# imisumi/software-path-tracer

Hardware: AMD Instinct MI355X
Metric: Msamples/sec (whole node), 1920x1080 x 8-bounce Cornell box (higher is better)
Workload: dtype f32

## Files before the change

include/spt.h:

```cpp
#ifndef SPT_H
#define SPT_H

#include <stddef.h>
#include <stdint.h>

#ifdef __cplusplus
extern "C" {
#endif

#define SPT_ABI_VERSION 3

typedef enum spt_status {
    SPT_OK = 0,
    SPT_ERR_INVALID = -1,
    SPT_ERR_HIP = -2,
    SPT_ERR_NO_DEVICE = -3,
    SPT_ERR_NO_SCENE = -4,
    SPT_ERR_NOT_CONFIGURED = -5,
    SPT_ERR_CAPACITY = -6
} spt_status;


typedef enum spt_prim_type {
    SPT_PRIM_SPHERE = 0,
// ... 40 lines not shown

typedef struct spt_config {
    uint32_t width;
    uint32_t height;
    uint32_t max_bounces;
    uint32_t rr_depth;
    uint32_t flags;
    uint32_t shard_rank;
    uint32_t shard_count;
    uint32_t frames_in_flight;
} spt_config;

#define SPT_MAX_BOUNCES 32
typedef struct spt_stats {
    uint64_t frames;
    uint64_t paths;
    uint64_t segments[SPT_MAX_BOUNCES];
    uint64_t segments_total;
    uint64_t passes;
    uint64_t extend_launches;
    double extend_ms;
    uint64_t extend_segments;
    uint64_t shade_launches;
    double shade_ms;
    double other_ms;
    double extend_ms_bounce[SPT_MAX_BOUNCES];
    double shade_ms_bounce[SPT_MAX_BOUNCES];
    uint64_t bvh_nodes;
    uint64_t scene_bytes;
    uint64_t radiance_updates[SPT_MAX_BOUNCES];
    double tail_ms;
    uint64_t tail_launches;
    uint64_t tail_bounce;
    uint64_t fused;
    double persistent_ms;
    uint64_t persistent_launches;
    uint64_t schedule;
    uint64_t lane_slots;
    uint64_t lane_busy;
    uint64_t bvh_node_visits;
    uint64_t prim_tests;
    uint64_t flat_fast_path;
    uint64_t specialized;
    uint64_t shadow_rays;
    uint64_t emitters;
    uint64_t stack_bytes;
    uint64_t stack_need;
    uint64_t stalled_waves;
    uint64_t view_cached;
    uint64_t view_live_pixels;
    uint64_t flat_pairs;
    uint64_t flat_pair_second_passes;
    uint64_t view_split;
} spt_stats;

typedef struct spt_ctx spt_ctx;

int spt_abi_version(void);
int spt_device_count(int* count);

int spt_create(spt_ctx** out, int device_id);
void spt_destroy(spt_ctx* ctx);
const char* spt_last_error(const spt_ctx* ctx);
int spt_set_stream(spt_ctx* ctx, void* hip_stream);

int spt_set_scene(spt_ctx* ctx, const spt_prim* prims, uint32_t n_prims,
                  const spt_material* mats, uint32_t n_mats, const spt_env* env);

int spt_update_prims(spt_ctx* ctx, const uint32_t* indices, const spt_prim* prims, uint32_t n);

int spt_configure(spt_ctx* ctx, const spt_config* cfg);
int spt_reset(spt_ctx* ctx);
int spt_get_frame_count(const spt_ctx* ctx, uint32_t* frame_count);

int spt_render(spt_ctx* ctx, uint32_t first_frame, uint32_t n_frames);
int spt_synchronize(spt_ctx* ctx);

int spt_shard_pixels(const spt_ctx* ctx, uint64_t* n_pixels);
int spt_read_accum(spt_ctx* ctx, float* host_rgba);
int spt_accum_device_ptr(spt_ctx* ctx, void** dptr, size_t* bytes);
int spt_copy_accum_device(spt_ctx* ctx, void* dst);
int spt_resolve_rgba8(spt_ctx* ctx, uint32_t frame_count, uint32_t* host_out);
int spt_resolve_rgba8_exposure(spt_ctx* ctx, uint32_t frame_count, float exposure, uint32_t* host_out);
int spt_register_host_output(spt_ctx* ctx, void* host_out, size_t bytes);
int spt_render_resolve_rgba8(spt_ctx* ctx, uint32_t first_frame, uint32_t n_frames, uint32_t frame_count,
                             float exposure, uint32_t* host_out);
int spt_assemble_rows(spt_ctx* ctx, const void* gathered, void* out);

#define SPT_CAMERA_JITTER 1u
typedef struct spt_camera {
    float origin[3], u[3], v[3], w[3];
    uint32_t flags;
    uint32_t reserved[3];
} spt_camera;
int spt_set_camera(spt_ctx* ctx, const spt_camera* camera);
int spt_camera_look_at(const float eye[3], const float target[3], const float up[3], float vfov_degrees,
                       spt_camera* out);
int spt_camera_ray(const spt_camera* camera, uint32_t width, uint32_t height, uint32_t x, uint32_t y,
                   float jx, float jy, float o[3], float d[3]);

typedef struct spt_lens {
    float radius;
    float focus_distance;
    uint32_t reserved[2];
} spt_lens;
int spt_set_camera_lens(spt_ctx* ctx, const spt_lens* lens);
// ... 91 lines not shown
```

software-path-tracer_amd/__init__.py:

```python
from __future__ import annotations

import ctypes
import enum
import os
from typing import Optional, Sequence, Tuple

import numpy as np

_HERE = os.path.dirname(os.path.abspath(__file__))
LIB_PATH = os.environ.get("SPT_LIB_PATH") or os.path.join(_HERE, "libspt_hip.so")
RENDER_LIB_PATH = os.path.join(_HERE, "libspt_render.so")

SPT_OK = 0
SPT_ERR = {
    -1: "SPT_ERR_INVALID",
    -2: "SPT_ERR_HIP",
    -3: "SPT_ERR_NO_DEVICE",
    -4: "SPT_ERR_NO_SCENE",
    -5: "SPT_ERR_NOT_CONFIGURED",
    -6: "SPT_ERR_CAPACITY",
}

PRIM_SPHERE, PRIM_QUAD, PRIM_TRIANGLE = 0, 1, 2
FLAG_ABS_FLOAT = 1
# ... 61 lines not shown
class SptLens(ctypes.Structure):
    _fields_ = [
        ("radius", ctypes.c_float),
        ("focus_distance", ctypes.c_float),
        ("reserved", ctypes.c_uint32 * 2),
    ]


CAMERA_JITTER = 1
SPT_MAX_BOUNCES = 32


class SptStats(ctypes.Structure):
    _fields_ = [
        ("frames", ctypes.c_uint64),
        ("paths", ctypes.c_uint64),
        ("segments", ctypes.c_uint64 * SPT_MAX_BOUNCES),
        ("segments_total", ctypes.c_uint64),
        ("passes", ctypes.c_uint64),
        ("extend_launches", ctypes.c_uint64),
        ("extend_ms", ctypes.c_double),
        ("extend_segments", ctypes.c_uint64),
        ("shade_launches", ctypes.c_uint64),
        ("shade_ms", ctypes.c_double),
        ("other_ms", ctypes.c_double),
        ("extend_ms_bounce", ctypes.c_double * SPT_MAX_BOUNCES),
        ("shade_ms_bounce", ctypes.c_double * SPT_MAX_BOUNCES),
        ("bvh_nodes", ctypes.c_uint64),
        ("scene_bytes", ctypes.c_uint64),
        ("radiance_updates", ctypes.c_uint64 * SPT_MAX_BOUNCES),
        ("tail_ms", ctypes.c_double),
        ("tail_launches", ctypes.c_uint64),
        ("tail_bounce", ctypes.c_uint64),
        ("fused", ctypes.c_uint64),
        ("persistent_ms", ctypes.c_double),
        ("persistent_launches", ctypes.c_uint64),
        ("schedule", ctypes.c_uint64),
        ("lane_slots", ctypes.c_uint64),
        ("lane_busy", ctypes.c_uint64),
        ("bvh_node_visits", ctypes.c_uint64),
        ("prim_tests", ctypes.c_uint64),
        ("flat_fast_path", ctypes.c_uint64),
        ("specialized", ctypes.c_uint64),
        ("shadow_rays", ctypes.c_uint64),
        ("emitters", ctypes.c_uint64),
        ("stack_bytes", ctypes.c_uint64),
        ("stack_need", ctypes.c_uint64),
        ("stalled_waves", ctypes.c_uint64),
        ("view_cached", ctypes.c_uint64),
        ("view_live_pixels", ctypes.c_uint64),
        ("flat_pairs", ctypes.c_uint64),
        ("flat_pair_second_passes", ctypes.c_uint64),
        ("view_split", ctypes.c_uint64),
    ]

    def as_dict(self) -> dict:
        d = {}
        for k, _ in self._fields_:
            v = getattr(self, k)
            d[k] = list(v) if isinstance(v, ctypes.Array) else v
        return d


EXPORTED_SYMBOLS = (
    "spt_abi_version", "spt_device_count", "spt_create", "spt_destroy", "spt_last_error", "spt_set_stream",
    "spt_set_scene", "spt_configure", "spt_reset", "spt_get_frame_count", "spt_render", "spt_synchronize",
    "spt_shard_pixels", "spt_read_accum", "spt_accum_device_ptr", "spt_copy_accum_device", "spt_resolve_rgba8",
    "spt_resolve_rgba8_exposure", "spt_register_host_output", "spt_render_resolve_rgba8", "spt_assemble_rows",
    "spt_set_profiling", "spt_get_stats", "spt_stats_clear", "spt_build_scene",
    "spt_set_env_map", "spt_env_octa_from_equirect",
    "spt_comm_available", "spt_comm_unique_id", "spt_comm_init", "spt_gather_image", "spt_gather_image_overlapped", "spt_gather_wait",
    "spt_comm_destroy", "spt_set_tuning",
    "spt_specialize_scene", "spt_compile_flat_kernels", "spt_update_prims",
    "spt_set_camera", "spt_camera_look_at", "spt_camera_ray",
    "spt_set_camera_lens", "spt_camera_lens_ray", "spt_camera_focus_at_hit",
    "spt_set_material_models", "spt_bsdf_sample",
    "spt_render_features", "spt_read_features", "spt_features_device_ptr",
    "spt_denoise_params_default", "spt_denoise", "spt_set_denoise_form", "spt_read_denoised", "spt_denoised_device_ptr",
    "spt_resolve_denoised_rgba8", "spt_atrous_host",
)
COMM_ID_BYTES = 128


class SptTuning(ctypes.Structure):
    _fields_ = [
        ("fused", ctypes.c_int32),
        ("tail_bounce", ctypes.c_uint32),
        ("persistent", ctypes.c_int32),
        ("frame_kernel", ctypes.c_int32),
        ("chunks_per_wave", ctypes.c_uint32),
        ("px_shift", ctypes.c_uint32),
        ("subqueues", ctypes.c_uint32),
        ("bvh_max_leaf", ctypes.c_uint32),
        ("bvh_bins", ctypes.c_uint32),
        ("specialize", ctypes.c_int32),
        ("view_cache", ctypes.c_int32),
        ("split_streams", ctypes.c_int32),
    ]

    def __init__(self, **kw):
        super().__init__(fused=-1, persistent=-1, frame_kernel=-1)
        for k, v in kw.items():
            if k not in dict(self._fields_):
                raise TypeError(f"unknown spt_tuning field {k}")
            setattr(self, k, v)

# ... 793 lines not shown
```

software-path-tracer_amd/csrc/spt_capi.hip:

```cpp
#include <dlfcn.h>
#include <hip/hip_runtime.h>
#include <rccl/rccl.h>

#include <algorithm>
#include <cmath>
#include <cstdio>
#include <cstdlib>
#include <cstring>
#include <string>
#include <vector>

#include "scene.h"
#include "spt.h"
#include "spt_denoise.h"
#include "spt_device.h"
#include "spt_jit.h"
#include "spt_kernels.h"
#include "spt_launch_plan.h"

using namespace spt;

static_assert(kBvhStackMax == kBvhStackEntries, "scene.h and spt_kernels.h stack bounds");
static_assert(kMatDiffuse == SPT_MAT_DIFFUSE && kMatMetal == SPT_MAT_METAL && kMatDielectric == SPT_MAT_DIELECTRIC,
              "spt.h spt_material_kind and spt_device.h model_kind");
// ... 1867 lines not shown
    return SPT_OK;
}

int spt_get_stats(spt_ctx* c, spt_stats* out) {
    if (!c || !out) return SPT_ERR_INVALID;
    SPT_HIP(c, hipSetDevice(c->device));
    SPT_HIP(c, hipStreamSynchronize(on_stream(c)));
    if (flush_events(c) != SPT_OK) return SPT_ERR_HIP;
    unsigned long long tot[kTotals];
    SPT_HIP(c, hipMemcpy(tot, c->totals, sizeof(tot), hipMemcpyDeviceToHost));
    std::memset(out, 0, sizeof(*out));
    out->frames = c->frames;
    out->paths = c->paths;
    out->passes = c->passes;
    for (uint32_t b = 0; b < kMaxBounces && b < SPT_MAX_BOUNCES; ++b) {
        out->segments[b] = tot[b];
        out->segments_total += tot[b];
        out->radiance_updates[b] = tot[kMaxBounces + b];
    }
    out->extend_launches = c->ext_launches;
    out->extend_ms = c->ext_ms;
    out->extend_segments = c->ext_launches ? out->segments_total : 0;
    out->shade_launches = c->shade_launches;
    out->shade_ms = c->shade_ms;
    out->other_ms = c->other_ms;
    out->tail_ms = c->tail_ms;
    out->tail_launches = c->tail_launches;
    out->tail_bounce = schedule_tail(c);
    out->fused = schedule_fused(c) ? 1u : 0u;
    out->persistent_ms = c->persist_ms;
    out->persistent_launches = c->persist_launches;
    out->schedule = c->last_schedule;
    out->lane_slots = tot[2 * kMaxBounces];
    out->lane_busy = tot[2 * kMaxBounces + 1];
    out->bvh_node_visits = tot[2 * kMaxBounces + 2];
    out->prim_tests = tot[2 * kMaxBounces + 3];
    out->flat_fast_path = (c->fast_div && c->n_prims <= kFlatSceneMax) ? 1u : 0u;
    out->specialized = c->last_specialized ? 1u : 0u;
    for (uint32_t b = 0; b < kMaxBounces && b < SPT_MAX_BOUNCES; ++b) {
        out->extend_ms_bounce[b] = c->ext_ms_b[b];
        out->shade_ms_bounce[b] = c->shade_ms_b[b];
    }
    out->bvh_nodes = c->n_nodes;
    out->scene_bytes = c->scene_bytes;
    out->shadow_rays = tot[kTotShadow];
    out->emitters = c->n_emit;
    out->stack_bytes = c->stack_bytes;
    out->stack_need = c->bvh_stack_need;
    out->stalled_waves = tot[kTotStalled];
    out->view_cached = c->last_view_cached ? 1u : 0u;
    out->view_live_pixels = c->view_valid ? c->view_n[0] : 0u;
    out->flat_pairs = c->last_specialized ? c->last_pairs : 0u;
    out->flat_pair_second_passes = tot[kTotPairSecond];
    out->view_split = c->last_view_split ? 1u : 0u;
    if (tot[kTotStalled])
        return fail(c, SPT_ERR_HIP, "k_paths: " + std::to_string(tot[kTotStalled]) +
                                        " wave(s) stopped at the step bound with frames unaccumulated (a bug)");
    return SPT_OK;
}

int spt_stats_clear(spt_ctx* c) {
    if (!c) return SPT_ERR_INVALID;
    SPT_HIP(c, hipSetDevice(c->device));
    SPT_HIP(c, hipStreamSynchronize(on_stream(c)));
    if (flush_events(c) != SPT_OK) return SPT_ERR_HIP;
    SPT_HIP(c, hipMemset(c->totals, 0, sizeof(unsigned long long) * kTotals));
    c->frames = c->paths = c->passes = 0;
    c->ext_launches = c->shade_launches = c->ext_segments = 0;
    c->ext_ms = c->shade_ms = c->other_ms = c->tail_ms = 0.0;
    c->tail_launches = 0;
    c->persist_ms = 0.0;
    c->persist_launches = 0;
    for (uint32_t b = 0; b < kMaxBounces; ++b) c->ext_ms_b[b] = c->shade_ms_b[b] = 0.0;
    return SPT_OK;
}

int spt_specialize_scene(spt_ctx* c) {
    if (!c) return SPT_ERR_INVALID;
    if (!c->has_scene) return fail(c, SPT_ERR_NO_SCENE, "spt_specialize_scene before spt_set_scene");
    if (c->n_prims == 0 || c->n_nodes != 0 || c->specialize < 0) return SPT_OK;
    SPT_HIP(c, hipSetDevice(c->device));
    const uint64_t key = flat_jit_key(c);
    std::string err;
    const JitKindList kinds = jit_kinds_of_scene(nee_active(c), c->d_env ? 1 : 0);
    for (int i = 0; i < kinds.n; ++i)
        if (!jit_function(kinds.k[i].kind, kinds.k[i].env, key, &err))
            return fail(c, SPT_ERR_HIP, ("specialized kernels unavailable (the generic ones run): " + err).c_str());
    return SPT_OK;
}

int spt_compile_flat_kernels(const spt_prim* prims, uint32_t n_prims, int env_map, char* log, size_t log_bytes) {
    if (log && log_bytes) log[0] = 0;
    if ((!prims && n_prims) || n_prims == 0 || n_prims > kFlatSceneMax) return SPT_ERR_INVALID;
    uint32_t n_mats = 1;
    for (uint32_t i = 0; i < n_prims; ++i) n_mats = std::max(n_mats, prims[i].material + 1u);
    std::vector<DevPrim> dp, sorted;
    const char* msg = nullptr;
    if (!prepare_prims(prims, n_prims, n_mats, dp, &msg)) return SPT_ERR_INVALID;
    uint32_t ends[kFlatKinds - 1], flat_ends = 0;
    sort_flat_by_kind(dp, sorted, ends);
    for (uint32_t g = 0; g + 1 < kFlatKinds; ++g) flat_ends |= ends[g] << (6 * g);
    const uint32_t flat_rect = flat_rect_bits(sorted, ends);
    const uint64_t key = flat_shape_key(flat_ends, n_prims, flat_rect, flat_wall_pairs(sorted, ends, flat_rect));
    std::string out;
    const JitKindList kinds = jit_kinds_of_scene(false, env_map ? 1 : 0);
    int built = 0;
// ... 180 lines not shown
```

software-path-tracer_amd/csrc/spt_device.h:

```cpp
#pragma once

#ifndef __HIPCC_RTC__
#include <hip/hip_runtime.h>
#include <stdint.h>
#else
typedef __hip_internal::uint8_t uint8_t;
typedef __hip_internal::uint16_t uint16_t;
typedef __hip_internal::uint32_t uint32_t;
typedef __hip_internal::uint64_t uint64_t;
typedef __hip_internal::int32_t int32_t;
#endif

namespace spt {

constexpr float kInf = __builtin_inff();
constexpr uint32_t kMiss = 0xffffffffu;
constexpr float kTNear = 0.001f;
constexpr float kOriginEps = 1e-4f;
constexpr float kPiF = 3.14159265358979323846f;
constexpr uint32_t kSeedPrime = 982451653u;
constexpr uint32_t kFlagAbsFloat = 1u;

struct F3 {
    float x, y, z;
// ... 287 lines not shown
    const float y = (float)((double)sin_t * sp);
#endif
    const float z = cos_t;
    const F3 b = cross3(n, t);
    return F3{(x * t.x + y * b.x) + z * n.x, (x * t.y + y * b.y) + z * n.y, (x * t.z + y * b.z) + z * n.z};
}

template <bool kSmemCoef = false>
__host__ __device__ __forceinline__ F3 bounce_dir(F3 n, uint32_t& state, uint32_t flags) {
    return bounce_dir_frame<kSmemCoef>(n, bounce_tangent(n, flags), state);
}


__device__ __forceinline__ float isect_sphere(float4 s, F3 o, F3 d, float tmin) {
    const float lx = o.x - s.x, ly = o.y - s.y, lz = o.z - s.z;
    const float a = (d.x * d.x + d.y * d.y) + d.z * d.z;
    const float b = 2.0f * ((lx * d.x + ly * d.y) + lz * d.z);
    const float c = ((lx * lx + ly * ly) + lz * lz) - s.w * s.w;
    const float disc = b * b - 4.0f * a * c;
    if (!(disc >= 0.0f)) return kInf;
    const float sq = sqrtf(disc);
    const float two_a = 2.0f * a;
    const float t1 = (-b - sq) / two_a;
    if (t1 >= tmin) return t1;
    const float t2 = (-b + sq) / two_a;
    if (t2 >= tmin) return t2;
    return kInf;
}

__device__ __forceinline__ F3 rr_divide(F3 T, float p) {
    auto in_range = [](float c) { return (c == 0.0f) | (c >= 0x1p-100f); };
    const bool p_ok = (p >= 0x1p-40f) & (p <= 0x1p20f);
    if ((p_ok & in_range(T.x) & in_range(T.y) & in_range(T.z))) {
        const RcpRef r = rcp_ref(p);
        return F3{div_ref(T.x, r), div_ref(T.y, r), div_ref(T.z, r)};
    }
    return F3{T.x / p, T.y / p, T.z / p};
}

__device__ __forceinline__ float isect_sphere_fast(float4 s, float rr, F3 o, F3 d, float a, RcpRef r2a, float tmin,
                                                   bool& redo) {
    const float lx = o.x - s.x, ly = o.y - s.y, lz = o.z - s.z;
    const float b = 2.0f * ((lx * d.x + ly * d.y) + lz * d.z);
    const float c = ((lx * lx + ly * ly) + lz * lz) - rr;
    const float disc = b * b - 4.0f * a * c;
    redo = redo | ((disc > 0.0f) & (disc < 0x1p-96f));
    if (!((disc >= 0x1p-96f) | (disc == 0.0f))) return kInf;
    const float sq = sqrt_unit(disc);
    const float t1 = div_ref(-b - sq, r2a);
    if (t1 >= tmin) return t1;
    const float t2 = div_ref(-b + sq, r2a);
    if (t2 >= tmin) return t2;
    return kInf;
}

__device__ __forceinline__ float comp(float4 v, int i) { return i == 0 ? v.x : (i == 1 ? v.y : v.z); }
__device__ __forceinline__ float comp(F3 v, int i) { return i == 0 ? v.x : (i == 1 ? v.y : v.z); }

template <int AX>
__device__ __forceinline__ float isect_quad_axis(float4 pa, float4 pb, float4 pc, float4 pd, F3 o, F3 d, float tmin) {
    constexpr int U = AX == 0 ? 1 : 0;
    constexpr int V = AX == 2 ? 1 : 2;
    (void)pb;
    const float t = (comp(pa, AX) - comp(o, AX)) / comp(d, AX);
    if (!(t >= tmin) || t == kInf) return kInf;
    const float hu = (comp(o, U) + t * comp(d, U)) - comp(pa, U);
    const float hv = (comp(o, V) + t * comp(d, V)) - comp(pa, V);
    const float al = hu * comp(pc, U) + hv * comp(pc, V);
    const float be = hu * comp(pd, U) + hv * comp(pd, V);
    const uint32_t ua = __float_as_uint(al + 0.0f), ub = __float_as_uint(be + 0.0f);
    return max(ua, ub) <= 0x3f800000u ? t : kInf;
}

template <int AX, bool kRect = false>
__device__ __forceinline__ float isect_quad_axis_fast(float4 pa, float4 pc, float4 pd, F3 o, F3 d, RcpRef rAX,
                                                      float tmin) {
    constexpr int U = AX == 0 ? 1 : 0;
    constexpr int V = AX == 2 ? 1 : 2;
    const float t = div_ref(comp(pa, AX) - comp(o, AX), rAX);
    const float hu = (comp(o, U) + t * comp(d, U)) - comp(pa, U);
    const float hv = (comp(o, V) + t * comp(d, V)) - comp(pa, V);
    float al, be;
    if (kRect || (((__float_as_uint(comp(pc, V)) | __float_as_uint(comp(pd, U))) & 0x7fffffffu) == 0u)) {
        al = hu * comp(pc, U);
        be = hv * comp(pd, V);
    } else {
        al = hu * comp(pc, U) + hv * comp(pc, V);
        be = hu * comp(pd, U) + hv * comp(pd, V);
    }
    const uint32_t ua = __float_as_uint(al + 0.0f), ub = __float_as_uint(be + 0.0f);
    return (t >= tmin && max(ua, ub) <= 0x3f800000u) ? t : kInf;
}

template <int AX>
__device__ __forceinline__ float isect_rect_axis_fast(float q, float qu, float qv, float cu, float dv, F3 o, F3 d,
                                                      RcpRef rAX, float tmin) {
    constexpr int U = AX == 0 ? 1 : 0;
    constexpr int V = AX == 2 ? 1 : 2;
    const float t = div_ref(q - comp(o, AX), rAX);
    const float hu = (comp(o, U) + t * comp(d, U)) - qu;
    const float hv = (comp(o, V) + t * comp(d, V)) - qv;
    const float al = hu * cu;
    const float be = hv * dv;
    const uint32_t ua = __float_as_uint(al + 0.0f), ub = __float_as_uint(be + 0.0f);
    return (t >= tmin && max(ua, ub) <= 0x3f800000u) ? t : kInf;
}
// ... 140 lines not shown
```

software-path-tracer_amd/csrc/spt_kernels.h:

```cpp
#pragma once

#ifndef __HIPCC_RTC__
#include <hip/hip_runtime.h>
#include <stdint.h>
#endif

namespace spt {

constexpr uint32_t kBlock = 256;
constexpr uint32_t kChunk = 64;
constexpr uint32_t kMaxBounces = 32;
constexpr uint32_t kFlagFastDiv = 1u << 30;
constexpr uint32_t kTotShadow = 2 * kMaxBounces + 4;
constexpr uint32_t kTotStalled = 2 * kMaxBounces + 5;
constexpr uint32_t kTotPairSecond = 2 * kMaxBounces + 6;
constexpr uint32_t kTotals = 2 * kMaxBounces + 7;

constexpr uint32_t kFlagNee = 1u << 4;
struct NeeParams {
    const float4* emit;
    uint32_t n_emit;
    uint32_t spheres;
};
constexpr int kNeeAll = 1;
constexpr int kNeeNoSpheres = 2;

struct QueueBufs {
    float4* o;
    float4* d;
    float4* t;
};

struct PassParams {
    const float4* prims;
    const float4* mats;
    const float4* nodes;
    uint32_t n_prims;
    uint32_t n_mats;
    uint32_t n_nodes;
    uint32_t n_dev_nodes;
    uint32_t sky_enabled;
    uint32_t flags;
    uint32_t flat_ends;
    float4 horizon;
    float4 zenith;
    const float4* env;
    uint32_t env_w, env_h;
    uint32_t width, height;
    uint32_t shard_rank, shard_count;
    uint32_t shard_pixels;
    float inv_w, inv_h, aspect;
    uint32_t max_bounces, rr_depth;
    uint32_t first_frame;
    uint32_t n_frames;
    uint32_t n_paths;
    uint32_t n_sub;
    uint32_t sub_cap;
    QueueBufs q[2];
    float2* hit;
    float4* radiance;
    float4* accum;
    uint32_t* counts;
    unsigned long long* totals;
    uint32_t* work;
    uint32_t* work_next;
    uint32_t cu_count;
    uint32_t chunks_per_wave;
    uint32_t px_shift;
    void* stack;
// ... 180 lines not shown
```

software-path-tracer_amd/csrc/spt_kernels.hip:

```cpp
#ifndef __HIPCC_RTC__
#include <algorithm>
#endif

#include "spt_device.h"
#include "spt_kernels.h"

namespace spt {

namespace {

__device__ __forceinline__ float isect_any(const float4* __restrict__ prims, uint32_t k, uint32_t type, F3 o, F3 d) {
    if (type == 0u) return isect_sphere(prims[4 * k + 0], o, d, kTNear);
    if (type == 1u) return isect_quad(prims[4 * k + 0], prims[4 * k + 1], prims[4 * k + 2], prims[4 * k + 3], o, d, kTNear);
    return isect_tri(prims[4 * k + 0], prims[4 * k + 1], prims[4 * k + 2], o, d, kTNear);
}

__device__ __forceinline__ void closest_flat_exact(const float4* __restrict__ prims, uint32_t n_prims, F3 o, F3 d,
                                                   float& best_t, uint32_t& best_k) {
    for (uint32_t k = 0; k < n_prims; ++k) {
        const float t = isect_any(prims, k, meta_type(prims[4 * k + 3]), o, d);
        if (t < best_t) {
            best_t = t;
            best_k = k;
        }
    }
}

#define SPT_PIN4(v) asm volatile("" ::"s"((v).x), "s"((v).y), "s"((v).z), "s"((v).w))


template <uint64_t kShape>
__device__ __forceinline__ void make_pair_table(const float4* __restrict__ prims, float4* tab) {
    constexpr uint32_t kEnds = (uint32_t)(kShape & 0x3fffffffu), kN = (uint32_t)(kShape >> 30) & 63u;
    constexpr uint32_t kE0 = 2u * flat_shape_pairs(kShape, 0u), kE1 = kE0 + 2u * flat_shape_pairs(kShape, 1u);
    constexpr uint32_t kE2 = kE1 + 2u * flat_shape_pairs(kShape, 2u);
    const uint32_t e = threadIdx.x;
    if (e < kE2) {
        const int ax = e < kE0 ? 0 : (e < kE1 ? 1 : 2);
        const int u = ax == 0 ? 1 : 0, v = ax == 2 ? 1 : 2;
        const uint32_t first = ax == 0 ? 0u : (ax == 1 ? kE0 : kE1);
        const uint32_t k = kN + ((kEnds >> (6 * ax)) & 63u) + (e - first);
        const float4 pa = prims[4 * k + 0], pb = prims[4 * k + 1], pc = prims[4 * k + 2], pd = prims[4 * k + 3];
        tab[2 * e + 0] = make_float4(comp(pa, ax), comp(pa, u), comp(pa, v), comp(pc, u));
        tab[2 * e + 1] = make_float4(comp(pd, v), pb.w, 0.0f, 0.0f);
    }
}

#ifndef SPT_PAIR_FORM
#define SPT_PAIR_FORM 0
#endif

template <int AX, uint32_t kNP>
__device__ __forceinline__ void flat_pair_tests(const float4* __restrict__ kp, const float4* tab, F3 o, F3 d, RcpRef r,
                                                uint64_t& best, uint32_t* second) {
    if constexpr (kNP != 0u) {
        constexpr int U = AX == 0 ? 1 : 0;
        constexpr int V = AX == 2 ? 1 : 2;
        const bool up = comp(d, AX) > 0.0f;
        const float oa = comp(o, AX);
        const float4* lane_tab = tab + (up ? 2 : 0);
        const float4* other_tab = tab + (up ? 0 : 2);
#pragma unroll
        for (uint32_t p = 0; p < kNP; ++p) {
            const float4 la = kp[8 * p + 0], ha = kp[8 * p + 4];
            auto test = [&](const float4* t4, bool high) {
#if SPT_PAIR_FORM == 1
                (void)t4;
                const float4 lb = kp[8 * p + 1], lc = kp[8 * p + 2], ld = kp[8 * p + 3];
                const float4 hb = kp[8 * p + 5], hc = kp[8 * p + 6], hd = kp[8 * p + 7];
                const float4 e0 = make_float4(high ? comp(ha, AX) : comp(la, AX), high ? comp(ha, U) : comp(la, U),
                                              high ? comp(ha, V) : comp(la, V), high ? comp(hc, U) : comp(lc, U));
                const float4 e1 = make_float4(high ? comp(hd, V) : comp(ld, V), high ? hb.w : lb.w, 0.0f, 0.0f);
#else
                (void)high;
                const float4 e0 = t4[4 * p + 0], e1 = t4[4 * p + 1];
#endif
                const float t = isect_rect_axis_fast<AX>(e0.x, e0.y, e0.z, e0.w, e1.x, o, d, r, kTNear);
                const uint64_t key = ((uint64_t)__float_as_uint(t) << 32) | __float_as_uint(e1.y);
                best = key < best ? key : best;
            };
            test(lane_tab, up);
            const bool inside = comp(la, AX) <= oa && oa <= comp(ha, AX);
            if (__ballot(!inside) != 0ull) {
                test(other_tab, !up);
                if (second && __lane_id() == (uint32_t)__ffsll((long long)__ballot(true)) - 1u) atomicAdd(second, 1u);
            }
        }
    }
}

#define SPT_NOPIN(v) ((void)0)
#define SPT_NOHEAD(AX, RD)
#define SPT_PAIR_HEAD(AX, RD)                                                                   \
    flat_pair_tests<AX, flat_shape_pairs(kShape, AX)>(kp + 4 * k, pair_tab + 4 * pair0, o, d, RD, best, second); \
    k += 2u * flat_shape_pairs(kShape, AX);                                                     \
    pair0 += flat_shape_pairs(kShape, AX);
#define SPT_FLAT_GROUPS(UNROLL, PIN, HEAD)                                                      \
    {                                                                                           \
        uint32_t k = 0;                                                                         \
        UNROLL for (const uint32_t e = flat_ends & 63u; k < e; ++k) {              \
            const float4 pa = kp[4 * k + 0], pb = kp[4 * k + 1];                                \
            PIN(pa);                                                                            \
            PIN(pb);                                                                            \
            take(isect_sphere_fast(pa, pb.x, o, d, a, r2a, kTNear, redo), pb);                  \
        }                                                                                       \
        HEAD(0, rdx)                                                                            \
        SPT_FLAT_GROUP(UNROLL, PIN, 6, (isect_quad_axis_fast<0, ((kRectBits >> 0) & 1u) != 0u>(pa, pc, pd, o, d, rdx, kTNear))) \
        HEAD(1, rdy)                                                                            \
        SPT_FLAT_GROUP(UNROLL, PIN, 12, (isect_quad_axis_fast<1, ((kRectBits >> 1) & 1u) != 0u>(pa, pc, pd, o, d, rdy, kTNear))) \
        HEAD(2, rdz)                                                                            \
        SPT_FLAT_GROUP(UNROLL, PIN, 18, (isect_quad_axis_fast<2, ((kRectBits >> 2) & 1u) != 0u>(pa, pc, pd, o, d, rdz, kTNear))) \
        SPT_FLAT_GROUP(UNROLL, PIN, 24, (isect_quad(pa, pb, pc, pd, o, d, kTNear)))              \
        UNROLL for (; k < n_prims; ++k) {                                        \
            const float4 pa = kp[4 * k + 0], pb = kp[4 * k + 1], pc = kp[4 * k + 2];            \
            PIN(pa);                                                                            \
            PIN(pb);                                                                            \
            PIN(pc);                                                                            \
            take(isect_tri(pa, pb, pc, o, d, kTNear), pb);                                      \
        }                                                                                       \
    }
#define SPT_FLAT_GROUP(UNROLL, PIN, SHIFT, TEST)                                                \
    UNROLL for (const uint32_t e = (flat_ends >> (SHIFT)) & 63u; k < e; ++k) {                  \
        const float4 pa = kp[4 * k + 0], pb = kp[4 * k + 1];                                    \
        const float4 pc = kp[4 * k + 2], pd = kp[4 * k + 3];                                    \
        PIN(pa);                                                                                \
        PIN(pb);                                                                                \
        PIN(pc);                                                                                \
        PIN(pd);                                                                                \
        take(TEST, pb);                                                                         \
    }

template <uint64_t kShape = 0, bool kPaired = false>
__device__ __forceinline__ void closest_flat(const float4* __restrict__ prims, uint32_t n_prims, F3 o, F3 d,
                                             float& best_t, uint32_t& best_k, bool fast_scene = false,
                                             uint32_t flat_ends = 0u, const float4* pair_tab = nullptr,
                                             uint32_t* second = nullptr) {
    const float in_t = best_t;
    const uint32_t in_k = best_k;
    constexpr uint32_t kRectBits = (uint32_t)(kShape >> 53) & 7u;
    if (fast_scene) {
        const float a = (d.x * d.x + d.y * d.y) + d.z * d.z;
        const float dmin = fminf(fminf(fabsf(d.x), fabsf(d.y)), fabsf(d.z));
        const bool ok = dmin >= 0x1p-20f && a >= 0.5f && a <= 2.0f;
        if (__ballot(!ok) == 0ull) {
            const RcpRef r2a = rcp_ref(2.0f * a);
            const RcpRef rdx = rcp_ref(d.x), rdy = rcp_ref(d.y), rdz = rcp_ref(d.z);
            bool redo = false;
            uint64_t best = ((uint64_t)__float_as_uint(in_t) << 32) | in_k;
            auto take = [&](float t, float4 pb) {
                const uint64_t key = ((uint64_t)__float_as_uint(t) << 32) | __float_as_uint(pb.w);
                best = key < best ? key : best;
            };
            if constexpr (kShape != 0) {
                const uint32_t flat_ends = (uint32_t)(kShape & 0x3fffffffu);
                const uint32_t n_prims = (uint32_t)(kShape >> 30) & 63u;
                const float4* __restrict__ kp = prims + 4 * n_prims;
                if constexpr (kPaired && flat_shape_pairs(kShape) != 0u) {
                    static_assert((((kShape >> 57) & 3u) == 0u || (kRectBits & 1u)) && (((kShape >> 59) & 3u) == 0u || (kRectBits & 2u)) &&
                                  (((kShape >> 61) & 3u) == 0u || (kRectBits & 4u)), "wall pairs only in rectangle groups");
                    uint32_t pair0 = 0;
                    SPT_FLAT_GROUPS(_Pragma("unroll"), SPT_NOPIN, SPT_PAIR_HEAD)
                } else {
                    SPT_FLAT_GROUPS(_Pragma("unroll"), SPT_NOPIN, SPT_NOHEAD)
                }
            } else {
                const float4* __restrict__ kp = prims + 4 * n_prims;
                SPT_FLAT_GROUPS(, SPT_PIN4, SPT_NOHEAD)
            }
            if (__ballot(redo) == 0ull || !redo) {
                best_t = __uint_as_float((uint32_t)(best >> 32));
                best_k = best == (((uint64_t)__float_as_uint(in_t) << 32) | in_k) ? in_k
                         : (best_t < kInf ? (uint32_t)best : kMiss);
                return;
            }
            best_t = in_t;
            best_k = in_k;
        }
    }
    closest_flat_exact(prims, n_prims, o, d, best_t, best_k);
}
#undef SPT_FLAT_GROUP
#undef SPT_FLAT_GROUPS
#undef SPT_NOPIN
#undef SPT_NOHEAD
#undef SPT_PAIR_HEAD

struct BvhCounters {
    uint32_t nodes = 0, prims = 0;
};

constexpr int kStack4 = kBvhStackEntries;

// ... 1041 lines not shown
__device__ __forceinline__ void advance_rays(const float4* __restrict__ nodes, const float4* __restrict__ prims,
                                             bool have, bool can_start, F3 o, F3 d, Trav& tv, bool& tdone,
                                             const Stk& stk, BvhCounters& ctr,
                                             uint32_t& lane_slots, uint32_t& lane_busy,
                                             const float4* top = nullptr, uint32_t n_top = 0u,
                                             const float4* ptop = nullptr, uint32_t n_ptop = 0u,
                                             uint32_t batch = kBvhBatch) {
    for (;;) {
        const bool trav = have && !tdone;
        const unsigned long long tm = __ballot(trav);
        if (tm == 0ull) break;
        if ((uint32_t)__popcll(__ballot(have ? tdone : can_start)) >= batch) break;
        if (kStats) {
            lane_slots += 64u;
            lane_busy += (uint32_t)__popcll(tm);
        }
        if (trav)
            tdone = trav_step<kStats, kLds, kAnyHit>(nodes, prims, o, d, tv, stk, &ctr, top, n_top, ptop, n_ptop);
    }
}

template <bool kStats, bool kBvh, int kEnv, uint64_t kShape = 0, int kSimdWaves = 0, bool kChan = false, int kNee = 0,
          bool kJitter = false, bool kBsdf = false>
__global__ __launch_bounds__(kBlock, kSimdWaves ? kSimdWaves : (kBvh ? kPathsWavesBvh : ((kNee || kBsdf) ? kPathsWaves : kPathsWavesFlat))) void k_paths(const float4* __restrict__ prims, const float4* __restrict__ mats,
                                                  const float4* __restrict__ nodes, uint32_t n_prims,
                                                  float4* __restrict__ accum,
                                                  unsigned long long* __restrict__ totals,
                                                  uint32_t* __restrict__ work, uint32_t* __restrict__ work_next,
                                                  ShadeParams sp, CameraParams cam, uint32_t n_frames, ChunkPlan plan,
                                                  NeeParams nee, ViewPlan view) {
    constexpr uint32_t kWaves = kBlock / 64u;
    constexpr bool kStart0 = kJitter || kBsdf;
    constexpr bool kView = !kBvh && !kStart0;
    bake_config<kShape>(sp);
    constexpr uint32_t kRingSlots = ring_slots<kBvh>();
    extern __shared__ float4 s_scene[];
    constexpr uint32_t kPxRecs = kBvh ? 3u : kFlatPxRecs;
    __shared__ float4 s_px[kWaves][kPxRecs][1u << kMaxChunkShift];
    __shared__ float s_L[kWaves][3][kRingSlots];
    __shared__ __attribute__((aligned(16))) uint32_t s_cnt[kWaves][64];
    __shared__ uint8_t s_pix[kWaves][1u << kMaxChunkShift];
    constexpr uint32_t kTop = kBvh ? (kSimdWaves == 8 ? kBvhTopNodes8 : kBvhTopNodes) : 0u;
    __shared__ float4 s_top[kTop ? 4u * kTop : 1u];
    const uint32_t n_top = min(kTop, sp.n_nodes);
    for (uint32_t k = threadIdx.x; k < 4u * n_top; k += kBlock) s_top[k] = nodes[k];
    __shared__ uint32_t s_seg[kStats ? kMaxBounces : 1u];
    __shared__ uint32_t s_rmw[kStats ? kMaxBounces : 1u];
    __shared__ uint32_t s_shadow[kStats && kNee ? 1u : 1u];
    if (kStats && kNee && threadIdx.x == 0u) s_shadow[0] = 0u;
    if (!kBvh) make_shade_recs(prims, mats, sp.n_prims, s_scene);
    constexpr uint32_t kPairs = kBvh ? 0u : flat_shape_pairs(kShape);
    [[maybe_unused]] float4* const pair_tab = s_scene + 3u * ((uint32_t)(kShape >> 30) & 63u);
    [[maybe_unused]] uint32_t* const pair_second = kStats ? (uint32_t*)(pair_tab + 4u * kPairs) : nullptr;
    if constexpr (kPairs != 0u) {
        make_pair_table<kShape>(prims, pair_tab);
        if (kStats && threadIdx.x == 0u) *pair_second = 0u;
    }
    if (blockIdx.x == 0u && threadIdx.x < kWorkHeads) work_next[threadIdx.x * kWorkStride] = 0u;
    if (kStats && threadIdx.x < kMaxBounces) {
        s_seg[threadIdx.x] = 0;
        s_rmw[threadIdx.x] = 0;
    }
    __syncthreads();
    const float4* sh_prims = kBvh ? prims : s_scene;
    const float4* sh_mats = mats;

    const uint32_t wave = __builtin_amdgcn_readfirstlane(threadIdx.x / 64u);
    const uint32_t lane = __lane_id();
    const auto stk = lane_stack<kSimdWaves == 8 ? kBvhStackEntry8W : kBvhStackEntry>(sp, blockIdx.x * kWaves + wave, lane);
    uint32_t lane_slots = 0, lane_busy = 0;
    BvhCounters bvh_ctr;
    uint32_t n_chunks = plan.n[0] + plan.n[1] + plan.n[2];
    bool view_on = false;
    if constexpr (kView) {
        view_on = view.live != nullptr;
        if (view_on) n_chunks += view.n_sweep;
    }
    const uint32_t xcc = xcc_id();
    uint32_t heads_empty = 0;
    constexpr bool kOrdered = true;
#ifdef SPT_TIMELINE
    const unsigned long long tl_start = wall_clock64();
    unsigned long long tl_last = tl_start;
    uint32_t tl_chunks = 0, tl_pxs = 0, tl_live = 0;
#endif
    for (;;) {
        uint32_t chunk = pull_unit(work, n_chunks, xcc, heads_empty);
        if (chunk >= n_chunks) break;
#ifdef SPT_TIMELINE
        tl_last = wall_clock64();
        ++tl_chunks;
#endif
        if constexpr (kView) {
            if (view_on && chunk >= plan.n[0]) {
                const uint32_t unit = chunk - plan.n[0];
                if (unit < view.n_sweep) {
                    const uint32_t i0 = unit * kViewSweep;
                    if (kStats && lane == 0u) atomicAdd(&s_seg[0], n_frames * min(kViewSweep, view.n_const - i0));
                    if (i0 + lane < view.n_const) {
                        const float4 c = view.constant[i0 + lane];
                        const uint32_t pix = __float_as_uint(c.w);
                        float4 a = accum[pix];
                        for (uint32_t f = 0; f < n_frames; ++f) a = make_float4(a.x + c.x, a.y + c.y, a.z + c.z, a.w);
                        a.w = add_count(a.w, n_frames);
                        accum[pix] = a;
                    }
#ifdef SPT_TIMELINE
                    tl_pxs = 6u;
                    tl_live = 0u;
// ... 516 lines not shown
                        fin_s = true;
                    }
                }
                finish(fin_s);
            }
        }
        if (steps_left == ~0u && lane == 0u) atomicAdd(&totals[kTotStalled], 1ull);
        if (kOrdered && plan.cost && chunk < plan.n[0] && lane == 0u)
            plan.cost[chunk] = (uint16_t)min(65535u, (kBvh && kNee) ? ((steps_init - steps_left) * 4u + titer) >> 2
                                                                    : steps_init - steps_left);
        if (ch_on) {
            uint32_t ap = pix0 + cp;
            if constexpr (kView) {
                if (view_on) ap = __float_as_uint(s_px[wave][2][cp].w);
            }
            float* af = reinterpret_cast<float*>(accum) + 4u * (size_t)ap + c0;
            af[0] = acc.x;
            if (pxs == kMaxChunkShift) af[1] = acc.y;
        } else if (!chmode && lane < npx) {
            uint32_t ap = pix0 + lane;
            if constexpr (kView) {
                if (view_on) ap = __float_as_uint(s_px[wave][2][lane].w);
            }
            accum[ap] = acc;
        }
    }
#ifdef SPT_TIMELINE
    if (lane == 0u) {
        unsigned long long* r = g_tl + 4u * (blockIdx.x * kWaves + wave);
        r[0] = tl_start;
        r[1] = tl_last;
        r[2] = wall_clock64();
        r[3] = tl_chunks | ((unsigned long long)xcc << 32) | ((unsigned long long)tl_pxs << 40) |
               ((unsigned long long)tl_live << 48);
    }
#endif
    if (kStats) {
        if (lane == 0u) {
            atomicAdd(&totals[2u * kMaxBounces], (unsigned long long)lane_slots);
            atomicAdd(&totals[2u * kMaxBounces + 1u], (unsigned long long)lane_busy);
        }
        if (kBvh) {
            atomicAdd(&totals[2u * kMaxBounces + 2u], (unsigned long long)bvh_ctr.nodes);
            atomicAdd(&totals[2u * kMaxBounces + 3u], (unsigned long long)bvh_ctr.prims);
        }
        __syncthreads();
        if (threadIdx.x < sp.max_bounces) {
            if (s_seg[threadIdx.x]) atomicAdd(&totals[threadIdx.x], (unsigned long long)s_seg[threadIdx.x]);
            if (s_rmw[threadIdx.x]) atomicAdd(&totals[kMaxBounces + threadIdx.x], (unsigned long long)s_rmw[threadIdx.x]);
        }
        if (kNee && threadIdx.x == 0u && s_shadow[0]) atomicAdd(&totals[kTotShadow], (unsigned long long)s_shadow[0]);
        if constexpr (kPairs != 0u)
            if (threadIdx.x == 0u && *pair_second) atomicAdd(&totals[kTotPairSecond], (unsigned long long)*pair_second);
    }
}

__device__ __forceinline__ uint32_t to_u8(float v, float frames) {
    float c = v / frames;
    c = c < 0.0f ? 0.0f : (1.0f < c ? 1.0f : c);
    if (c != c) c = 0.0f;
    return (uint32_t)(uint8_t)(c * 255.0f);
}

__device__ __forceinline__ uint32_t to_u8(float v, float frames, float exposure) {
    float c = v / frames;
    c = c * exposure;
    c = c < 0.0f ? 0.0f : (1.0f < c ? 1.0f : c);
    if (c != c) c = 0.0f;
    return (uint32_t)(uint8_t)(c * 255.0f);
}

__device__ __forceinline__ uint32_t rgba8(float4 a, float frames, float exposure) {
    return (to_u8(a.x, frames, exposure) << 24) | (to_u8(a.y, frames, exposure) << 16) |
           (to_u8(a.z, frames, exposure) << 8) | to_u8(a.w, frames);
}

constexpr uint32_t kFrameBvhBatch = 24;
constexpr uint32_t kFrameBvhBatchLds = 64;

template <bool kStats, bool kBvh, int kEnv, uint64_t kShape = 0, bool kSmall = false, int kNee = 0, bool kRgba = false,
          bool kBsdf = false>
__global__ __launch_bounds__(kBlock, kSmall ? kFrameWavesSmall : (kBvh ? kPathsWavesBvh : kPathsWaves)) void k_frame(const float4* __restrict__ prims, const float4* __restrict__ mats,
                                                  const float4* __restrict__ nodes, uint32_t n_prims,
                                                  float4* __restrict__ accum,
                                                  unsigned long long* __restrict__ totals,
                                                  uint32_t* __restrict__ work, uint32_t* __restrict__ work_next,
                                                  ShadeParams sp, CameraParams cam, NeeParams nee) {
    bake_config<kShape>(sp);
    if (blockIdx.x == 0u && threadIdx.x < kWorkHeads) work_next[threadIdx.x * kWorkStride] = 0u;
    const bool lists = cam.hit_mode == 3u;
    const uint32_t sky_blocks = lists ? cam.sky_blocks : 0u;
    if (blockIdx.x < sky_blocks) {
        const uint32_t n_sky = __builtin_amdgcn_readfirstlane(cam.list_counts[1]);
        for (uint32_t i = blockIdx.x * kBlock + threadIdx.x; i < n_sky; i += sky_blocks * kBlock) {
            const uint32_t px = cam.sky_pix[i];
            const CameraRay cr = camera_ray<kShape, false>(cam, px);
            float4 a = accum[px];
            F3 lc{0.f, 0.f, 0.f};
            if (sp.sky_enabled) {
                const F3 sky = sky_radiance<kEnv>(sp, cr.d);
                lc = F3{0.0f + 1.0f * sky.x, 0.0f + 1.0f * sky.y, 0.0f + 1.0f * sky.z};
            }
            a.x = a.x + lc.x;
            a.y = a.y + lc.y;
            a.z = a.z + lc.z;
            a.w = a.w + 1.0f;
// ... 875 lines not shown
```

Before: 127,600.

## Intersect few flat-scene spheres in one pass with a single sqrt per candidate

For flat scenes with 2-4 spheres, per-sphere intersection with a sqrt and division each is replaced by a pass that computes the discriminants for all spheres, picks the first candidate sphere per lane, and computes roots only for it. A second candidate gets its own root evaluation. If three or more candidates occur anywhere in the wave, it falls back to the full per-sphere test. Wave-wide ballots skip the second root when no lane needs it. This removes repeated sqrt/div work and adds a stats counter for second passes, at the cost of extra ballots and selection logic.

```diff
diff --git a/include/spt.h b/include/spt.h
--- a/include/spt.h
+++ b/include/spt.h
@@ -116,6 +116,7 @@
     uint64_t flat_pairs;
     uint64_t flat_pair_second_passes;
     uint64_t view_split;
+    uint64_t flat_sphere_second_passes;
 } spt_stats;
 
 typedef struct spt_ctx spt_ctx;
diff --git a/software-path-tracer_amd/__init__.py b/software-path-tracer_amd/__init__.py
--- a/software-path-tracer_amd/__init__.py
+++ b/software-path-tracer_amd/__init__.py
@@ -137,6 +137,7 @@
         ("flat_pairs", ctypes.c_uint64),
         ("flat_pair_second_passes", ctypes.c_uint64),
         ("view_split", ctypes.c_uint64),
+        ("flat_sphere_second_passes", ctypes.c_uint64),
     ]
 
     def as_dict(self) -> dict:
diff --git a/software-path-tracer_amd/csrc/spt_capi.hip b/software-path-tracer_amd/csrc/spt_capi.hip
--- a/software-path-tracer_amd/csrc/spt_capi.hip
+++ b/software-path-tracer_amd/csrc/spt_capi.hip
@@ -1943,6 +1943,7 @@
     out->view_live_pixels = c->view_valid ? c->view_n[0] : 0u;
     out->flat_pairs = c->last_specialized ? c->last_pairs : 0u;
     out->flat_pair_second_passes = tot[kTotPairSecond];
+    out->flat_sphere_second_passes = tot[kTotSphereSecond];
     out->view_split = c->last_view_split ? 1u : 0u;
     if (tot[kTotStalled])
         return fail(c, SPT_ERR_HIP, "k_paths: " + std::to_string(tot[kTotStalled]) +
diff --git a/software-path-tracer_amd/csrc/spt_device.h b/software-path-tracer_amd/csrc/spt_device.h
--- a/software-path-tracer_amd/csrc/spt_device.h
+++ b/software-path-tracer_amd/csrc/spt_device.h
@@ -363,6 +363,88 @@
     const float t2 = div_ref(-b + sq, r2a);
     if (t2 >= tmin) return t2;
     return kInf;
+}
+
+template <uint32_t kNS>
+__device__ __forceinline__ void flat_sphere_pass(const float4* __restrict__ kp, F3 o, F3 d, float a, RcpRef r2a, float tmin,
+                                                 bool& redo, uint64_t& best, uint32_t* second) {
+    auto roots = [&](float sb, float sdisc, uint32_t sidx, bool on, uint64_t lanes) {
+        const float sq = sqrt_unit(sdisc);
+        float t = div_ref(-sb - sq, r2a);
+        const bool low = !(t >= tmin);
+        if ((__builtin_amdgcn_ballot_w64(low) & lanes) != 0ull) {
+            asm volatile("" ::: "memory");
+            t = low ? div_ref(-sb + sq, r2a) : t;
+        }
+        t = (on & (t >= tmin)) ? t : kInf;
+        const uint64_t key = ((uint64_t)__float_as_uint(t) << 32) | sidx;
+        best = key < best ? key : best;
+    };
+    float bk[kNS], dk[kNS];
+    uint32_t ik[kNS];
+    bool cand[kNS];
+    uint64_t any = 0ull, many = 0ull, more = 0ull;
+#pragma unroll
+    for (uint32_t k = 0; k < kNS; ++k) {
+        const float4 s = kp[4 * k + 0], pb = kp[4 * k + 1];
+        const float lx = o.x - s.x, ly = o.y - s.y, lz = o.z - s.z;
+        const float b = 2.0f * ((lx * d.x + ly * d.y) + lz * d.z);
+        const float c = ((lx * lx + ly * ly) + lz * lz) - pb.x;
+        const float disc = b * b - 4.0f * a * c;
+        redo = redo | ((disc > 0.0f) & (disc < 0x1p-96f));
+        cand[k] = ((disc >= 0x1p-96f) | (disc == 0.0f)) & (!(b > 0.0f) | !(c > 0.0f));
+        bk[k] = b;
+        dk[k] = disc;
+        ik[k] = __float_as_uint(pb.w);
+        const uint64_t cm = (__builtin_amdgcn_ballot_w64(disc >= 0x1p-96f) | __builtin_amdgcn_ballot_w64(disc == 0.0f)) &
+                            (__builtin_amdgcn_ballot_w64(!(b > 0.0f)) | __builtin_amdgcn_ballot_w64(!(c > 0.0f)));
+        more |= cm & many;
+        many |= cm & any;
+        any |= cm;
+    }
+    float sb = bk[kNS - 1u], sdisc = dk[kNS - 1u];
+    uint32_t sidx = ik[kNS - 1u];
+    bool seen = cand[kNS - 1u];
+#pragma unroll
+    for (uint32_t k = kNS - 1u; k-- > 0u;) {
+        sb = cand[k] ? bk[k] : sb;
+        sdisc = cand[k] ? dk[k] : sdisc;
+        sidx = cand[k] ? ik[k] : sidx;
+        seen = seen | cand[k];
+    }
+    roots(sb, sdisc, sidx, seen, any);
+    if (many != 0ull) {
+        bool one = cand[0], two = false;
+        bool next[kNS];
+        next[0] = false;
+#pragma unroll
+        for (uint32_t k = 1; k < kNS; ++k) {
+            next[k] = cand[k] & one & !two;
+            two = two | (cand[k] & one);
+            one = one | cand[k];
+        }
+        float sb2 = bk[kNS - 1u], sdisc2 = dk[kNS - 1u];
+        uint32_t sidx2 = ik[kNS - 1u];
+#pragma unroll
+        for (uint32_t k = kNS - 1u; k-- > 1u;) {
+            sb2 = next[k] ? bk[k] : sb2;
+            sdisc2 = next[k] ? dk[k] : sdisc2;
+            sidx2 = next[k] ? ik[k] : sidx2;
+        }
+        roots(sb2, sdisc2, sidx2, two, many);
+        if (second && __lane_id() == (uint32_t)__ffsll((long long)__ballot(true)) - 1u) atomicAdd(second + 1, 1u);
+        if constexpr (kNS >= 3u) {
+            if (more != 0ull) {
+#pragma unroll
+                for (uint32_t k = 0; k < kNS; ++k) {
+                    const float4 s = kp[4 * k + 0], pb = kp[4 * k + 1];
+                    const float tk = isect_sphere_fast(s, pb.x, o, d, a, r2a, tmin, redo);
+                    const uint64_t kk = ((uint64_t)__float_as_uint(tk) << 32) | __float_as_uint(pb.w);
+                    best = kk < best ? kk : best;
+                }
+            }
+        }
+    }
 }
 
 __device__ __forceinline__ float comp(float4 v, int i) { return i == 0 ? v.x : (i == 1 ? v.y : v.z); }
diff --git a/software-path-tracer_amd/csrc/spt_kernels.h b/software-path-tracer_amd/csrc/spt_kernels.h
--- a/software-path-tracer_amd/csrc/spt_kernels.h
+++ b/software-path-tracer_amd/csrc/spt_kernels.h
@@ -14,7 +14,9 @@
 constexpr uint32_t kTotShadow = 2 * kMaxBounces + 4;
 constexpr uint32_t kTotStalled = 2 * kMaxBounces + 5;
 constexpr uint32_t kTotPairSecond = 2 * kMaxBounces + 6;
-constexpr uint32_t kTotals = 2 * kMaxBounces + 7;
+constexpr uint32_t kTotSphereSecond = 2 * kMaxBounces + 7;
+constexpr uint32_t kOnePassMax = 4;
+constexpr uint32_t kTotals = 2 * kMaxBounces + 8;
 
 constexpr uint32_t kFlagNee = 1u << 4;
 struct NeeParams {
diff --git a/software-path-tracer_amd/csrc/spt_kernels.hip b/software-path-tracer_amd/csrc/spt_kernels.hip
--- a/software-path-tracer_amd/csrc/spt_kernels.hip
+++ b/software-path-tracer_amd/csrc/spt_kernels.hip
@@ -27,7 +27,6 @@
 }
 
 #define SPT_PIN4(v) asm volatile("" ::"s"((v).x), "s"((v).y), "s"((v).z), "s"((v).w))
-
 
 template <uint64_t kShape>
 __device__ __forceinline__ void make_pair_table(const float4* __restrict__ prims, float4* tab) {
@@ -98,11 +97,16 @@
 #define SPT_FLAT_GROUPS(UNROLL, PIN, HEAD)                                                      \
     {                                                                                           \
         uint32_t k = 0;                                                                         \
-        UNROLL for (const uint32_t e = flat_ends & 63u; k < e; ++k) {              \
-            const float4 pa = kp[4 * k + 0], pb = kp[4 * k + 1];                                \
-            PIN(pa);                                                                            \
-            PIN(pb);                                                                            \
-            take(isect_sphere_fast(pa, pb.x, o, d, a, r2a, kTNear, redo), pb);                  \
+        if constexpr (kOnePass) {  \
+            flat_sphere_pass<(uint32_t)(kShape & 63u)>(kp, o, d, a, r2a, kTNear, redo, best, second); \
+            k = (uint32_t)(kShape & 63u);                                                       \
+        } else {                                                                                \
+            UNROLL for (const uint32_t e = flat_ends & 63u; k < e; ++k) {          \
+                const float4 pa = kp[4 * k + 0], pb = kp[4 * k + 1];                            \
+                PIN(pa);                                                                        \
+                PIN(pb);                                                                        \
+                take(isect_sphere_fast(pa, pb.x, o, d, a, r2a, kTNear, redo), pb);              \
+            }                                                                                   \
         }                                                                                       \
         HEAD(0, rdx)                                                                            \
         SPT_FLAT_GROUP(UNROLL, PIN, 6, (isect_quad_axis_fast<0, ((kRectBits >> 0) & 1u) != 0u>(pa, pc, pd, o, d, rdx, kTNear))) \
@@ -138,6 +142,7 @@
     const float in_t = best_t;
     const uint32_t in_k = best_k;
     constexpr uint32_t kRectBits = (uint32_t)(kShape >> 53) & 7u;
+    [[maybe_unused]] constexpr bool kOnePass = kShape != 0 && kPaired && (kShape & 63u) >= 2u && (kShape & 63u) <= kOnePassMax;
     if (fast_scene) {
         const float a = (d.x * d.x + d.y * d.y) + d.z * d.z;
         const float dmin = fminf(fminf(fabsf(d.x), fabsf(d.y)), fabsf(d.z));
@@ -1285,9 +1290,11 @@
     constexpr uint32_t kPairs = kBvh ? 0u : flat_shape_pairs(kShape);
     [[maybe_unused]] float4* const pair_tab = s_scene + 3u * ((uint32_t)(kShape >> 30) & 63u);
     [[maybe_unused]] uint32_t* const pair_second = kStats ? (uint32_t*)(pair_tab + 4u * kPairs) : nullptr;
+    constexpr bool kCountSpheres = kStats && kPairs != 0u && (kShape & 63u) >= 2u && (kShape & 63u) <= kOnePassMax;
     if constexpr (kPairs != 0u) {
         make_pair_table<kShape>(prims, pair_tab);
         if (kStats && threadIdx.x == 0u) *pair_second = 0u;
+        if (kCountSpheres && threadIdx.x == 0u) pair_second[1] = 0u;
     }
     if (blockIdx.x == 0u && threadIdx.x < kWorkHeads) work_next[threadIdx.x * kWorkStride] = 0u;
     if (kStats && threadIdx.x < kMaxBounces) {
@@ -1910,6 +1917,8 @@
         if (kNee && threadIdx.x == 0u && s_shadow[0]) atomicAdd(&totals[kTotShadow], (unsigned long long)s_shadow[0]);
         if constexpr (kPairs != 0u)
             if (threadIdx.x == 0u && *pair_second) atomicAdd(&totals[kTotPairSecond], (unsigned long long)*pair_second);
+        if constexpr (kCountSpheres)
+            if (threadIdx.x == 0u && pair_second[1]) atomicAdd(&totals[kTotSphereSecond], (unsigned long long)pair_second[1]);
     }
 }
 
```

New measurement: 130,900, median of 6. 2.6% higher.
